# fanxiaochen/Multi-View-Registration

Hardware: AMD Instinct MI355X
Metric: ICP correspondences/sec + ms/iteration, 12-view x 200k pts (higher is better)
Workload: dtype f32

## Files before the change

multi-view-registration_amd/csrc/mvr_ctx.hip:

```cpp
#include <algorithm>
#include <chrono>
#include <cfloat>
#include <cmath>
#include <cstdio>
#include <cstring>

#include "mvr_internal.h"

namespace mvr {

int set_error(Ctx *c, int status, const char *what, hipError_t e)
{
  if (c) {
    c->last_error = what ? what : "";
    if (e != hipSuccess) { c->last_error += ": "; c->last_error += hipGetErrorString(e); }
  }
  return status;
}

void host_mark(const char *what)
{
  static const bool on = std::getenv("MVR_TRACE_HOST") != nullptr;
  if (!on) return;
  using namespace std::chrono;
// ... 922 lines not shown
    if (b > s.n) b = s.n;
    if (n > s.n - b) n = s.n - b;
    if (t.n == 0) n = 0;
    qb[k] = b; qn[k] = n;
    off_s[k + 1] = off_s[k] + s.n; off_t[k + 1] = off_t[k] + t.n;
    off_p[k + 1] = off_p[k] + (size_t)reduce_blocks_for(c, n) * 29;
  }
  const nnkey_t *keys_before = w->bkeys;
  if (int rc = ensure(w, w->bkeys, w->bkeys_cap, off_s[n_pairs])) return rc;
  if (int rc = ensure(w, w->brkeys, w->brkeys_cap, off_t[n_pairs])) return rc;
  const uint32_t *bound_before = w->bbound;
  if (int rc = ensure(w, w->bbound, w->bbound_cap, off_t[n_pairs])) return rc;
  if (w->bbound != bound_before) w->bbound_clean = false;
  if (int rc = ensure(w, w->bpartials, w->bpartials_cap, off_p[n_pairs])) return rc;
  if (int rc = ensure(w, w->blist, w->blist_cap, off_t[n_pairs])) return rc;
  if (int rc = ensure(w, w->bslot, w->bslot_cap, off_t[n_pairs])) return rc;
  std::vector<size_t> off_c((size_t)n_pairs + 1, 0);
  for (int k = 0; k < n_pairs; ++k) off_c[k + 1] = off_c[k] + (c->slots[dst[k]].n + 255) / 256;
  if (int rc = ensure(w, w->bchunks, w->bchunks_cap, off_c[n_pairs] + (size_t)n_pairs)) return rc;
  uint32_t *counts = w->bchunks + off_c[n_pairs];
  const double max2 = max_dist * max_dist;
  const float cap2 = cap_from_max2(max2);
  if ((phases & 2) && c->last_batch.size() >= (size_t)(pair_base + n_pairs))
    for (int k = 0; k < n_pairs; ++k) {
      BatchPairRec &r = c->last_batch[(size_t)(pair_base + k)];
      r.w = w; r.off_s = off_s[k]; r.off_t = off_t[k]; r.qb = qb[k]; r.qn = qn[k]; r.src = src[k]; r.dst = dst[k]; r.max2 = max2; r.reciprocal = reciprocal;
      r.src_set = c->slots[src[k]].set_id; r.dst_set = c->slots[dst[k]].set_id;
    }
  std::vector<unsigned long long> sig;
  sig.push_back((unsigned long long)n_pairs); sig.push_back((unsigned long long)(fma != 0));
  for (int k = 0; k < n_pairs; ++k) {
    const Cloud &s = c->slots[src[k]], &t = c->slots[dst[k]];
    const unsigned long long v[6] = {s.set_id, t.set_id, (unsigned long long)s.n, (unsigned long long)t.n, (unsigned long long)qb[k], (unsigned long long)qn[k]};
    sig.insert(sig.end(), v, v + 6);
  }
  const bool seed = c->seed_forward && (phases & 1) && keys_before == w->bkeys && w->fused_sig == sig;
  if (phases & 1) w->fused_sig = sig;
  std::vector<CullPair> fwd((size_t)n_pairs), rev((size_t)n_pairs);
  for (int k = 0; k < n_pairs; ++k) {
    const Cloud &s = c->slots[src[k]], &t = c->slots[dst[k]];
    fwd[k] = make_cull_pair(s, qb[k], qn[k], nullptr, t, w->bkeys + off_s[k]);
    fwd[k].key_by_pos = 1;
    fwd[k].seed_from_keys = seed ? 1u : 0u;
    rev[k] = make_cull_pair(t, 0, std::min(qn[k], t.n), nullptr, s, w->brkeys + off_t[k]);
    rev[k].qlist = w->blist + off_t[k]; rev[k].qcount = counts + k;
    rev[k].qbound = w->bbound + off_t[k];
  }
  bool grid_ok = c->ring_search != 0 && cap2 < FLT_MAX;
  for (int k = 0; k < n_pairs && grid_ok; ++k) {
    const Cloud &s = c->slots[src[k]], &t = c->slots[dst[k]];
    if (qn[k] == 0) continue;
    grid_ok = s.grid && t.grid && s.gcoords_valid && t.gcoords_valid && s.grid->n == s.n && t.grid->n == t.n &&
              s.order && t.order && s.grid->built_for == s.order.get() && t.grid->built_for == t.order.get();
  }
  std::vector<GridPair> gfwd, grev;
  if (grid_ok) {
    if (int rc = ensure(w, w->bheavy, w->bheavy_cap, off_s[n_pairs] + off_t[n_pairs])) return rc;
    if (int rc = ensure(w, w->bwide, w->bwide_cap, off_s[n_pairs] + off_t[n_pairs])) return rc;
    if (!w->bwide_count) {
      MVR_MAY_BLOCK(w, "the wide-query counters are not allocated yet");
      MVR_HIP_TRY(w, hipMalloc(&w->bwide_count, 3 * kWideCounters * sizeof(uint32_t)));
      MVR_HIP_TRY(w, hipMemsetAsync(w->bwide_count, 0, 3 * kWideCounters * sizeof(uint32_t), w->stream));
    }
    if (int rc = ensure(w, w->bcull_sets, w->bcull_sets_cap, off_s[n_pairs] / 64 + (size_t)n_pairs)) return rc;
    if (n_pairs > kWideCounters) grid_ok = false;
  }
  if (grid_ok) {
    gfwd.resize((size_t)n_pairs); grev.resize((size_t)n_pairs);
    for (int k = 0; k < n_pairs; ++k) {
      const Cloud &s = c->slots[src[k]], &t = c->slots[dst[k]];
      if (qn[k] == 0) { gfwd[k] = GridPair(); grev[k] = GridPair(); continue; }
      gfwd[k] = make_grid_pair(s, qb[k], qn[k], t, w->bkeys + off_s[k]);
      gfwd[k].key_by_pos = 1; gfwd[k].seed_from_keys = seed ? 1u : 0u; gfwd[k].mark = fwd[k].mark;
      gfwd[k].heavy = w->bheavy + off_s[k];
      grev[k] = make_grid_pair(t, 0, std::min(qn[k], t.n), s, w->brkeys + off_t[k]);
      grev[k].qlist = rev[k].qlist; grev[k].qcount = rev[k].qcount; grev[k].qbound = rev[k].qbound;
      grev[k].heavy = w->bheavy + off_s[n_pairs] + off_t[k];
      if (c->cull_list) { gfwd[k].cull_sets = w->bcull_sets + off_s[k] / 64 + (size_t)k; gfwd[k].cull_count = w->bwide_count + 2 * kWideCounters + k; }
      if (c->grid_wide) {
        grev[k].heavy = nullptr;
        gfwd[k].wide_list = w->bwide + off_s[k]; gfwd[k].wide_count = w->bwide_count + k;
        grev[k].wide_list = w->bwide + off_s[n_pairs] + off_t[k]; grev[k].wide_count = w->bwide_count + kWideCounters + k;
      }
    }
  }
  const bool grid_fwd = grid_ok && (seed || c->unseeded_grid);
  bool sets_on_grid = grid_ok && c->cull_list && c->grid_sets;
  if (sets_on_grid && c->grid_sets == 1)
    for (int k = 0; k < n_pairs && sets_on_grid; ++k) {
      if (!qn[k]) continue;
      const double span = (2.0 * max_dist + 4.0) / (double)c->slots[dst[k]].grid->h;
// ... 53 lines not shown
  for (int base = 0; base < n_pairs; base += kBatchPairs) {
    const int m = std::min(kBatchPairs, n_pairs - base);
    GlueBatch gb;
    gb.max2 = max2; gb.reciprocal = recip ? 1 : 0;
    for (int k = 0; k < 3; ++k) gb.origin[k] = origin[k];
    for (int j = 0; j < m; ++j) {
      const int k = base + j;
      const Cloud &s = c->slots[src[k]], &t = c->slots[dst[k]];
      GluePair &g = gb.p[j];
      g.src = s.pts; g.tgt = t.pts; g.qs = s.sorted; g.ts = t.sorted; g.by_pos = 1;
      if (s.sorted_stale) { g.qraw = s.lean_raw; g.qrec = s.pose_dev; }
      if (t.sorted_stale) { g.traw = t.lean_raw; g.trec = t.pose_dev; }
      g.keys = w->bkeys + off_s[k]; g.rkeys = w->brkeys + off_t[k];
      g.qperm = (s.order && qn[k]) ? s.order->perm : nullptr; g.tinv = (t.order && qn[k]) ? t.order->inv : nullptr;
      g.bound = w->bbound + off_t[k];
      g.list = w->blist + off_t[k]; g.slot = w->bslot + off_t[k]; g.chunks = w->bchunks + off_c[k]; g.qcount = counts + k;
      g.nt = qn[k] ? t.n : 0;
      g.partials = w->bpartials + off_p[k]; g.out = table + (size_t)k * 32;
      g.q_begin = qb[k]; g.q_count = qn[k]; g.blocks = reduce_blocks_for(c, qn[k]);
      if (grid_ok) { g.zero_a = w->bwide_count + k; g.zero_b = w->bwide_count + kWideCounters + k; g.zero_c = w->bwide_count + 2 * kWideCounters + k; }
    }
    if (recip) {
      if (!w->marked_in_search) { if (int rc = launch_flag_matched_batch(w, gb, m)) return rc; }
      if (int rc = launch_compact_flags_batch(w, gb, m)) return rc;
      if (grid_ok) {
        if (int rc = launch_nn_grid_batch(w, grev.data() + base, m, cap2, fma != 0)) return rc;
        if (c->grid_debug && c->grid_wide) {
          MVR_MAY_BLOCK(c, "grid_debug reads counters back");
          std::vector<uint32_t> cnt((size_t)2 * kWideCounters), qc((size_t)n_pairs);
          MVR_HIP_TRY(w, hipStreamSynchronize(w->stream));
          MVR_HIP_TRY(w, hipMemcpy(cnt.data(), w->bwide_count, cnt.size() * sizeof(uint32_t), hipMemcpyDeviceToHost));
// ... 151 lines not shown
  if (s.set_id != r.src_set || t.set_id != r.dst_set || !s.order || !t.order)
    return set_error(c, MVR_E_ARG, "the clouds of that pair have changed since the batch");
  MVR_HIP_TRY(c, hipSetDevice(c->device));
  if (r.qn == 0) return MVR_OK;
  Ctx *w = r.w;
  const size_t ns = s.n, nt = t.n;
  std::vector<nnkey_t> keys(r.qn), rkeys(nt);
  std::vector<uint32_t> slot(nt), sperm(ns), tperm(nt);
  MVR_HIP_TRY(c, hipStreamSynchronize(c->stream));
  if (w != c) MVR_HIP_TRY(c, hipStreamSynchronize(w->stream));
  MVR_HIP_TRY(c, hipMemcpy(keys.data(), w->bkeys + r.off_s + r.qb, r.qn * sizeof(nnkey_t), hipMemcpyDeviceToHost));
  MVR_HIP_TRY(c, hipMemcpy(sperm.data(), s.order->perm, ns * 4, hipMemcpyDeviceToHost));
  MVR_HIP_TRY(c, hipMemcpy(tperm.data(), t.order->perm, nt * 4, hipMemcpyDeviceToHost));
  if (r.reciprocal) {
    MVR_HIP_TRY(c, hipMemcpy(rkeys.data(), w->brkeys + r.off_t, nt * sizeof(nnkey_t), hipMemcpyDeviceToHost));
    MVR_HIP_TRY(c, hipMemcpy(slot.data(), w->bslot + r.off_t, nt * 4, hipMemcpyDeviceToHost));
  }
  struct Rec { int32_t q, mt; uint32_t d; };
  std::vector<Rec> acc;
  for (size_t p = 0; p < r.qn; ++p) {
    const nnkey_t key = keys[p];
    const uint32_t tpos = (uint32_t)key, db = (uint32_t)(key >> 32);
    float d; std::memcpy(&d, &db, 4);
    if (tpos == kNone || tpos >= nt || (double)d > r.max2) continue;
    const uint32_t qi = sperm[r.qb + p];
    if (r.reciprocal) {
      const uint32_t li = slot[tpos];
      if (li >= nt) continue;
      const nnkey_t rk = rkeys[li];
      const uint32_t rb = (uint32_t)(rk >> 32);
      float dr; std::memcpy(&dr, &rb, 4);
      if ((uint32_t)rk != qi || (double)dr > r.max2) continue;
    }
    acc.push_back(Rec{(int32_t)qi, (int32_t)tperm[tpos], db});
  }
  std::sort(acc.begin(), acc.end(), [](const Rec &a, const Rec &b) { return a.q < b.q; });
  for (size_t i = 0; i < acc.size() && i < cap; ++i) {
    if (query) query[i] = acc[i].q;
    if (match) match[i] = acc[i].mt;
    if (dist2) std::memcpy(&dist2[i], &acc[i].d, 4);
  }
  *m = acc.size();
// ... 869 lines not shown

API int mvr_ctx_tune(mvr_ctx *ctx, const char *key, int value)
{
  if (!ctx || !key) return MVR_E_ARG;
  Ctx *c = CTX(ctx);
  c->lean_route = false;
  if (!std::strcmp(key, "nn_q")) c->nn_q = value;
  else if (!std::strcmp(key, "nn_sub")) c->nn_sub = value;
  else if (!std::strcmp(key, "nn_blocks_per_cu")) c->nn_blocks_per_cu = value;
  else if (!std::strcmp(key, "nn_mode")) c->nn_mode = value;
  else if (!std::strcmp(key, "cull_q")) c->cull_q = value;
  else if (!std::strcmp(key, "cull_w")) c->cull_w = value;
  else if (!std::strcmp(key, "cull_slices")) c->cull_slices = value;
  else if (!std::strcmp(key, "seed_forward")) c->seed_forward = value != 0;
  else if (!std::strcmp(key, "lean_pose")) { if (value < 0 || value > 1) return MVR_E_ARG; c->lean_pose = value; }
  else if (!std::strcmp(key, "lazy_super")) { if (value < 0 || value > 1) return MVR_E_ARG; c->lazy_super = value; }
  else if (!std::strcmp(key, "fused_mark")) { if (value < 0 || value > 2) return MVR_E_ARG; c->fused_mark = value; }
  else if (!std::strcmp(key, "ring_search")) c->ring_search = value;
  else if (!std::strcmp(key, "seq_search")) { if (value < 0 || value > 1) return MVR_E_ARG; c->seq_search = value; }
  else if (!std::strcmp(key, "unseeded_grid")) { if (value < 0 || value > 1) return MVR_E_ARG; c->unseeded_grid = value; }
  else if (!std::strcmp(key, "seq_cell_points")) { if (value < 1) return MVR_E_ARG; c->seq_cell_points = value; }
  else if (!std::strcmp(key, "seq_seed")) {
    c->seq_seed = value != 0;
    if (!c->seq_seed) {
      MVR_HIP_TRY(c, hipStreamSynchronize(c->stream));
      for (auto &kv : c->seq_seeds) if (kv.second.d) (void)hipFree(kv.second.d);
      c->seq_seeds.clear();
    }
  }
  else if (!std::strcmp(key, "grid_light_rows")) { if (value < 1) return MVR_E_ARG; c->grid_light_rows = value; }
// ... 57 lines not shown
{
  if (!ctx || !n || cap < 0 || (cap && !ms)) return MVR_E_ARG;
  Ctx *c = CTX(ctx);
  *n = (int)c->pass_ms.size();
  for (int k = 0; k < cap && k < *n; ++k) ms[k] = c->pass_ms[(size_t)k];
  return MVR_OK;
}

API int mvr_ctx_stat(mvr_ctx *ctx, const char *key, double *value)
{
  if (!ctx || !key || !value) return MVR_E_ARG;
  Ctx *c = CTX(ctx);
  if (!std::strcmp(key, "piped_passes")) *value = (double)c->piped_passes;
  else if (!std::strcmp(key, "fused_passes")) *value = (double)c->fused_passes;
  else if (!std::strcmp(key, "lean_passes")) *value = (double)c->lean_passes;
  else if (!std::strcmp(key, "blocking_events")) *value = (double)c->blocking_events;
  else if (!std::strcmp(key, "pipeline")) *value = (double)c->pipeline;
  else if (!std::strcmp(key, "prerej_match_ms")) *value = c->prerej_ms[0];
  else if (!std::strcmp(key, "prerej_hypotheses_ms")) *value = c->prerej_ms[1];
  else if (!std::strcmp(key, "prerej_score_ms")) *value = c->prerej_ms[2];
  else if (!std::strncmp(key, "stage_", 6) && c->stage_stat) {
    unsigned long long h[64] = {0};
    std::vector<unsigned long long> raw(64 * 64);
    MVR_HIP_TRY(c, hipStreamSynchronize(c->stream));
    MVR_HIP_TRY(c, hipMemcpy(raw.data(), c->stage_stat, raw.size() * sizeof(unsigned long long), hipMemcpyDeviceToHost));
    for (int sh = 0; sh < 64; ++sh) for (int k = 0; k < 64; ++k) h[k] += raw[(size_t)sh * 64 + k];
    if (!std::strncmp(key, "stage_raw_", 10)) { const int k = std::atoi(key + 10); if (k < 0 || k > 63) return MVR_E_ARG; *value = (double)h[k]; }
    else if (!std::strcmp(key, "stage_staged")) *value = (double)(h[1] + h[9]);
    else if (!std::strcmp(key, "stage_rows")) *value = (double)(h[2] + h[10]);
    else if (!std::strcmp(key, "stage_width")) *value = (double)(h[3] + h[11]);
// ... 92 lines not shown
```

multi-view-registration_amd/csrc/mvr_cull.hip:

```cpp
#include "mvr_internal.h"

namespace mvr {
namespace {

constexpr int kSub = 32;
constexpr int kGrpPitch = 65;

template <bool FMA>
__device__ __forceinline__ float dist2(const float4 t, float qx, float qy, float qz)
{
  const float dx = t.x - qx, dy = t.y - qy, dz = t.z - qz;
  if (FMA) return __builtin_fmaf(dz, dz, __builtin_fmaf(dy, dy, dx * dx));
  float r = dx * dx;
  r = r + dy * dy;
  r = r + dz * dz;
  return r;
}

__device__ __forceinline__ float box_dist2(const float qlo[3], const float qhi[3], const float4 lo, const float4 hi)
{
  const float dx = fmaxf(0.f, fmaxf(lo.x - qhi[0], qlo[0] - hi.x));
  const float dy = fmaxf(0.f, fmaxf(lo.y - qhi[1], qlo[1] - hi.y));
  const float dz = fmaxf(0.f, fmaxf(lo.z - qhi[2], qlo[2] - hi.z));
  return dx * dx + dy * dy + dz * dz;
// ... 39 lines not shown
}

#ifdef MVR_STAMP
#define MVR_CLK() __builtin_readcyclecounter()
#else
#define MVR_CLK() 0ull
#endif

template <bool FMA, int Q, int W>
__device__ __forceinline__ void
nn_cull_body(const float4 *__restrict__ qs, uint32_t q_begin, uint32_t q_count, const uint8_t *__restrict__ qflags,
               const uint32_t *__restrict__ qlist, const uint32_t *__restrict__ qcount, const float4 *__restrict__ ts, uint32_t nt,
               const float4 *__restrict__ tlo, const float4 *__restrict__ thi, const float4 *__restrict__ cbox,
               const float4 *__restrict__ sbox, uint32_t n_tiles, float cap2, nnkey_t *__restrict__ keys, uint32_t key_by_pos,
               const uint32_t *__restrict__ qbound, uint32_t seed_from_keys, uint32_t *__restrict__ mark, uint32_t set,
               unsigned long long *__restrict__ evals)
{
  constexpr int NQ = 4 * Q;
  constexpr int NB = 64 * Q;
  static_assert(W == 1 || W == 2 || W == 4, "waves per query set");
  static_assert(4 * NB * sizeof(nnkey_t) <= 4 * kGrpPitch * sizeof(float4), "partials must fit the tile buffers");
  __shared__ float4 lds[W][4 * kGrpPitch];
  __shared__ unsigned sbest[NB];
  const int lane = threadIdx.x & 63, wv = __builtin_amdgcn_readfirstlane((int)(threadIdx.x >> 6));
  const int g = lane >> 4, l16 = lane & 15;
  const unsigned long long st_entry = MVR_CLK();
#ifdef MVR_TRACE
  const unsigned long long tr_rt0 = __builtin_amdgcn_s_memrealtime();
  unsigned long long trm[8] = {0, 0, 0, 0, 0, 0, 0, 0};
  unsigned trq = 0, tr_open = 0, tr_exp = 0;
  unsigned long long tr_t_open = 0, tr_t_exp = 0, tr_t_next = 0;
// ... 468 lines not shown
#pragma unroll 1
          for (int p = 0; p < 4 * W; ++p) {
            nnkey_t k;
            if constexpr (W == 1) k = (nnkey_t)__shfl(((nnkey_t)__float_as_uint(best[j]) << 32) | bsub[j], p * 16 + l16, 64);
            else k = part[p * NB + i];
            if ((uint32_t)(k >> 32) == dbits && (uint32_t)k != sub && (uint32_t)k != kNone)
              ow = min(ow, span_argmin<FMA, kSub / 4>(ts, nt, (uint32_t)k * kSub + g * (kSub / 4), d, fqx[j], fqy[j], fqz[j]));
          }
        }
      }
      ow = min(ow, (winner_t)__shfl_xor(ow, 16, 64));
      ow = min(ow, (winner_t)__shfl_xor(ow, 32, 64));
      if (g == 0 && pos < nq && (!qflags || qflags[q_begin + pos] != 0)) {
        uint32_t ord = (qlist || (qflags && !key_by_pos)) ? pos : q_begin + pos;
        if (!(qflags || qlist) && !key_by_pos) ord = (W == 1) ? __float_as_uint(qs[q_begin + pos].w) : fqw[j];
        const uint32_t low = key_by_pos ? (uint32_t)ow : (uint32_t)(ow >> 32);
        keys[ord] = (found && ow != kNoWinner) ? (((nnkey_t)dbits << 32) | low) : kKeyInit;
        if (mark && found && ow != kNoWinner) __hip_atomic_store(&mark[low], dbits, __ATOMIC_RELAXED, __HIP_MEMORY_SCOPE_AGENT);
      }
    }
    __builtin_amdgcn_sched_barrier(0);
  }
  MVR_MARK(7);
  if (evals && lane == 0) {
    const unsigned long long e = (unsigned long long)cells_done * 64ull * nvalid;
    unsigned long long *a = evals + (size_t)(set & (kEvalShards - 1)) * kEvalStride;
    unsigned long long *b = a + kEvalRegion;
    atomicAdd(a, e);
    atomicAdd(b, e);
    atomicMax(b + 1, (unsigned long long)cells_done);
// ... 40 lines not shown
#endif
#ifdef MVR_CULL_WAVES_MAX
#define MVR_CULL_WAVES_ATTR MVR_CULL_WAVES, MVR_CULL_WAVES_MAX
#else
#define MVR_CULL_WAVES_ATTR MVR_CULL_WAVES
#endif
template <bool FMA, int Q, int W>
__global__ void __launch_bounds__(64 * W) __attribute__((amdgpu_waves_per_eu(Q == 1 ? (W == 4 ? MVR_CULL_WAVES + 1 : MVR_CULL_WAVES) : 3)))
nn_cull_kernel(CullBatch batch, XcdMap map, unsigned long long *__restrict__ evals)
{
  uint32_t pair = 0, set = 0;
  if (!xcd_map_block(map, blockIdx.x, &pair, &set)) return;
  pair = (uint32_t)__builtin_amdgcn_readfirstlane((int)pair); set = (uint32_t)__builtin_amdgcn_readfirstlane((int)set);
  const CullPair &a = batch.p[pair];
  nn_cull_body<FMA, Q, W>(a.qs, a.q_begin, a.q_count, a.qflags, a.qlist, a.qcount, a.ts, a.nt, a.tlo, a.thi, a.cbox, a.sbox, a.n_tiles, batch.cap2,
                          a.keys, a.key_by_pos, a.qbound, a.seed_from_keys, a.key_by_pos ? a.mark : nullptr, set, evals);
}

template <bool FMA, int W>
__global__ void __launch_bounds__(64 * W)
nn_cull_list_kernel(CullBatch batch, unsigned long long *__restrict__ evals)
{
  const CullPair &a = batch.p[blockIdx.y];
  if (!a.setcount) return;
  const uint32_t n = *a.setcount;
  for (uint32_t i = blockIdx.x; i < n; i += gridDim.x) {
    const uint32_t set = (uint32_t)__builtin_amdgcn_readfirstlane((int)a.setlist[i]);
    nn_cull_body<FMA, 1, W>(a.qs, a.q_begin, a.q_count, a.qflags, a.qlist, a.qcount, a.ts, a.nt, a.tlo, a.thi, a.cbox, a.sbox, a.n_tiles, batch.cap2,
                            a.keys, a.key_by_pos, a.qbound, a.seed_from_keys, a.key_by_pos ? a.mark : nullptr, set, evals);
    __syncthreads();
  }
}

}

int launch_nn_cull_list_batch(Ctx *c, const CullPair *pairs, int n_pairs, float cap2, bool fma)
{
  if (int rc = flush_super_boxes(c)) return rc;
  for (int base = 0; base < n_pairs; base += kBatchPairs) {
    CullBatch batch;
    const int m = std::min(kBatchPairs, n_pairs - base);
    bool any = false;
    for (int k = 0; k < kBatchPairs; ++k) {
      batch.p[k] = k < m ? pairs[base + k] : CullPair{};
// ... 127 lines not shown
```

multi-view-registration_amd/csrc/mvr_grid.hip:

```cpp
#include <hipcub/hipcub.hpp>

#include <algorithm>
#include <cmath>
#include <cstring>
#include <iterator>
#include <type_traits>
#include <vector>

#include "mvr_internal.h"
#include "mvr_grid_size.h"

namespace mvr {

CellGrid::~CellGrid()
{
  if (block) (void)hipFree(block);
  if (ready) (void)hipEventDestroy(ready);
}

namespace {

struct GridGeom { float lo[3]; float inv_h; int dim[3]; };

__device__ __forceinline__ int cell_of(float x, float lo, float inv_h, int dim)
// ... 510 lines not shown
        }
      }
    }
    if (stage_stat && lane == 0 && why) atomicAdd(stage_stat + (size_t)((blockIdx.x * 4u + (uint32_t)wv) & 63u) * 64u + why + (a.qlist ? 8u : 0u), 1ull);
    if (staged) walks = false;
  }
#ifdef MVR_STAGE_CLOCK
  if (!staged) { while (ckn < 4) { ck[ckn] = (long long)__builtin_readcyclecounter(); ++ckn; } }
#endif
  if (walks) walk_box(x0, x1, y0, y1, z0, z1);
  MVR_CK();
  if (answers) {
    const float bd = __uint_as_float((uint32_t)(best >> 32));
    const uint32_t bi = (uint32_t)best;
    const bool found = bi != kNone && bd <= cap2;
    const uint32_t ord = a.qlist ? pos : (a.key_by_pos ? qpos : __float_as_uint(q.w));
    uint32_t low = bi;
    if (found && (a.key_by_pos || a.mark)) {
      const uint32_t hp = a.tinv[bi];
      if (a.key_by_pos) low = hp;
      if (a.mark) __hip_atomic_store(&a.mark[hp], __float_as_uint(bd), __ATOMIC_RELAXED, __HIP_MEMORY_SCOPE_AGENT);
    }
    a.keys[ord] = found ? (((nnkey_t)__float_as_uint(bd) << 32) | low) : kKeyInit;
  }
  if (a.cull_sets) {
    if (__ballot(went_cull) != 0ull && (threadIdx.x & 63) == 0) a.cull_sets[atomicAdd(a.cull_count, 1u)] = (set * kGridThreads + threadIdx.x) >> 6;
  }
  {
    const unsigned long long m = __ballot(went_wide);
    if (m) {
      const int lane = threadIdx.x & 63;
// ... 81 lines not shown
        const nnkey_t key = ((nnkey_t)__float_as_uint(gdist2<FMA>(t, q.x, q.y, q.z)) << 32) | __float_as_uint(t.w);
        if (key < best) { best = key; bk = k; }
      }
      n_eval += total;
      __builtin_amdgcn_fence(__ATOMIC_RELEASE, "wavefront"); __builtin_amdgcn_wave_barrier(); __builtin_amdgcn_fence(__ATOMIC_ACQUIRE, "wavefront");
    }
    nnkey_t m = best;
#pragma unroll
    for (int o = 32; o > 0; o >>= 1) { const nnkey_t v = (nnkey_t)__shfl_xor((unsigned long long)m, o, 64); m = v < m ? v : m; }
    const unsigned long long who = __ballot(best == m && (uint32_t)best != kNone);
    const bool found = (uint32_t)m != kNone && __uint_as_float((uint32_t)(m >> 32)) <= cap2;
    if (found && who) {
      const int src = __ffsll((long long)who) - 1;
      const uint32_t wk = (uint32_t)__shfl((int)bk, src, 64);
      if (lane == 0) {
        const uint32_t ord = a.qlist ? pos : (a.key_by_pos ? qpos : __float_as_uint(q.w));
        uint32_t low = (uint32_t)m;
        if (a.key_by_pos || a.mark) {
          const uint32_t hp = a.g2h[wk];
          if (a.key_by_pos) low = hp;
          if (a.mark) __hip_atomic_store(&a.mark[hp], (uint32_t)(m >> 32), __ATOMIC_RELAXED, __HIP_MEMORY_SCOPE_AGENT);
        }
        a.keys[ord] = (m & 0xFFFFFFFF00000000ull) | low;
      }
    } else if (lane == 0) {
      const uint32_t ord = a.qlist ? pos : (a.key_by_pos ? qpos : __float_as_uint(q.w));
      a.keys[ord] = kKeyInit;
    }
  }
  if (evals && lane == 0 && n_eval) {
    unsigned long long *s = evals + (size_t)((bx * kWideWaves + wv) & (kEvalShards - 1)) * kEvalStride;
    atomicAdd(s, n_eval);
    atomicAdd(s + kEvalRegion, n_eval);
  }
}

}

namespace {
size_t align256(size_t v) { return (v + 255) & ~(size_t)255; }
__global__ void bbox_many_partial_kernel(const float4 *const *__restrict__ pts, const unsigned long long *__restrict__ n, float *__restrict__ part)
// ... 815 lines not shown
```

multi-view-registration_amd/csrc/mvr_index.hip:

```cpp
#include <hipcub/hipcub.hpp>

#include <algorithm>
#include <cstring>
#include <vector>

#include "mvr_internal.h"

namespace mvr {

uint32_t *OrderPool::take(size_t bytes, size_t *got)
{
  int best = -1;
  for (int k = 0; k < (int)free.size(); ++k)
    if (free[k].bytes >= bytes && free[k].bytes <= 4 * bytes + (1u << 20) && (best < 0 || free[k].bytes < free[best].bytes)) best = k;
  if (best < 0) return nullptr;
  uint32_t *p = free[best].p;
  *got = free[best].bytes;
  free.erase(free.begin() + best);
  return p;
}

void OrderPool::give(uint32_t *p, size_t bytes)
{
  if (!p) return;
// ... 337 lines not shown
  if (lane == 0) wsum[wave] = wave_all;
  __syncthreads();
  unsigned before = 0, all = 0;
#pragma unroll
  for (int w = 0; w < kChunk / 64; ++w) { if (w < wave) before += wsum[w]; all += wsum[w]; }
  *total = all;
  return before + mine;
}

__device__ __forceinline__ void chunk_write(const GluePair &a, const unsigned m, const size_t base, const unsigned first)
{
#pragma unroll
  for (int j = 0; j < kChunkPer; ++j)
    if ((m >> j) & 1u) {
      const unsigned at = first + (unsigned)__popc(m & ((1u << j) - 1u));
      a.list[at] = (uint32_t)(base + j); a.slot[base + j] = at;
    }
}

__global__ void __launch_bounds__(kChunk) count_flags_batch_kernel(GlueBatch b)
{
  const GluePair &a = b.p[blockIdx.y];
  if ((size_t)blockIdx.x * kChunkPos >= a.nt) return;
  unsigned total;
  (void)chunk_rank(flagged4(a, (size_t)blockIdx.x * kChunkPos + (size_t)threadIdx.x * kChunkPer), &total);
  if (threadIdx.x == 0) a.chunks[blockIdx.x] = total;
}

constexpr int kScanThreads = 1024;
__global__ void __launch_bounds__(kScanThreads) scan_chunks_batch_kernel(GlueBatch b)
{
// ... 629 lines not shown
```

multi-view-registration_amd/csrc/mvr_internal.h:

```cpp
#pragma once

#include <hip/hip_runtime.h>

#include <algorithm>
#include <cstddef>
#include <cstdint>
#include <map>
#include <memory>
#include <string>
#include <unordered_map>
#include <vector>

#include "mvr_hip.h"

namespace mvr {
hipError_t pool_malloc(void **p, size_t bytes);
hipError_t pool_free(void *p);
hipError_t pool_host_malloc(void **p, size_t bytes, unsigned flags);
hipError_t pool_host_free(void *p);
template <class T> inline hipError_t pool_malloc_t(T **p, size_t bytes) { return pool_malloc(reinterpret_cast<void **>(p), bytes); }
template <class T> inline hipError_t pool_host_malloc_t(T **p, size_t bytes, unsigned flags = 0) { return pool_host_malloc(reinterpret_cast<void **>(p), bytes, flags); }
template <class T> inline hipError_t pool_free_t(T *p) { return pool_free(const_cast<void *>(static_cast<const void *>(p))); }
template <class T> inline hipError_t pool_host_free_t(T *p) { return pool_host_free(const_cast<void *>(static_cast<const void *>(p))); }
}
// ... 97 lines not shown

using nnkey_t = unsigned long long;
constexpr nnkey_t kKeyInit = ~0ull;

constexpr int kNNThreads = 256;
constexpr int kNNTile = 1024;

constexpr int kCullTile = 256;
constexpr int kEvalShards = 64, kEvalStride = 16;
constexpr size_t kEvalRegion = (size_t)kEvalShards * kEvalStride;
constexpr size_t kTraceBlocks = 4096, kTraceRec = 16;

struct ProfRec { int family; hipEvent_t a, b; double work; const uint64_t *h_count; int n_shards; double per_count; };

struct Ctx;
struct BatchPairRec { Ctx *w = nullptr; size_t off_s = 0, off_t = 0, qb = 0, qn = 0; int src = -1, dst = -1; double max2 = 0.0; int reciprocal = 0; unsigned long long src_set = 0, dst_set = 0; };

struct Ctx {
  int device = 0;
  hipStream_t stream = nullptr;
  bool own_stream = false;
  int n_cu = 0;
  struct Cloud *refresh_rider = nullptr;
  int reduce_rows = 0;
  int clock_mhz = 0;
  std::string name;
  std::string last_error;
  Cloud slots[MVR_MAX_SLOTS + 2];
  uint64_t next_set_id = 1;
  std::map<uint64_t, std::weak_ptr<Order> > orders;
  std::map<uint64_t, std::weak_ptr<CellGrid> > grids;
// ... 98 lines not shown
  uint32_t *done_counter = nullptr; uint32_t signal_seq = 0; bool signal_armed = false, signal_sent = false;
  int lazy_super = 1;
  int setup_first = 1;
  int pose_prep_launch = 0;
  const double *pose_in_cur = nullptr; PoseRec *pose_tab_cur = nullptr; int pose_tab_n = 0; bool pose_tab_pending = false;
  uint32_t *gate = nullptr; bool gate_is_signal = false;
  uint32_t *h_done = nullptr, *d_done = nullptr;
  bool pipe_ops_warm = false;
  uint32_t pipe_seq = 0;
  unsigned long long pipe_steady_sig = 0, pipe_steady_events = ~0ull;
  std::vector<double> pass_ms;
  unsigned long long piped_passes = 0;
  int lean_pose = 1;
  bool lean_route = false;
  unsigned long long lean_passes = 0;
  void *comm = nullptr; bool comm_owned = false; int comm_rank = 0, comm_world = 1;
  void **comm_lender = nullptr;
  bool stream_stuck = false;
  bool comm_broken = false;
  int project_world = 0, project_rank = 0;
  double *proj_rows = nullptr; size_t proj_rows_cap = 0, proj_rows_n = 0;
  int wait_timeout_ms = 60000;
  long long dist_pass = 0, inject_fail_at = -1, inject_stall_at = -1;
  uint32_t *h_stall = nullptr, *d_stall = nullptr;
  long long *seq_keys = nullptr; size_t seq_keys_cap = 0;
  double *seq_row = nullptr;
  double *dist_table = nullptr; size_t dist_table_cap = 0;
  bool prof = false;
  unsigned prof_mask = ~0u;
  bool prof_totals = false;
// ... 150 lines not shown
int flush_super_boxes(Ctx *c);
void new_point_set(Ctx *c, Cloud &cl);
void inherit_point_set(Cloud &dst, const Cloud &src);
bool extend_point_set(Ctx *c, Cloud &dst, size_t old_n, const Cloud &src);
constexpr int kBatchPairs = 16;
struct CullPair {
  const float4 *qs = nullptr, *ts = nullptr, *tlo = nullptr, *thi = nullptr, *cbox = nullptr, *sbox = nullptr;
  const uint8_t *qflags = nullptr;
  const uint32_t *qlist = nullptr, *qcount = nullptr;
  nnkey_t *keys = nullptr;
  uint32_t q_begin = 0, q_count = 0, nt = 0, n_tiles = 0;
  const uint32_t *qbound = nullptr;
  uint32_t *mark = nullptr;
  uint32_t key_by_pos = 0;
  uint32_t seed_from_keys = 0;
  const uint32_t *setlist = nullptr, *setcount = nullptr;
};
struct CullBatch { CullPair p[kBatchPairs]; float cap2; };
CullPair make_cull_pair(const Cloud &q, size_t q_begin, size_t q_count, const uint8_t *qflags, const Cloud &t, nnkey_t *keys);
struct XcdMap { uint32_t sets[kBatchPairs]; uint32_t n_pairs, slices; };
__host__ __device__ inline uint32_t slice_len(uint32_t sets, uint32_t slices, uint32_t slice)
{
  return sets > slice ? (sets - slice + slices - 1u) / slices : 0u;
}
__host__ __device__ inline bool xcd_map_block(const XcdMap &m, uint32_t block, uint32_t *pair, uint32_t *set)
{
  uint32_t r = block >> 3;
  for (uint32_t u = block & 7u; u < m.n_pairs * m.slices; u += 8u) {
    const uint32_t p = u / m.slices, sl = u % m.slices, len = slice_len(m.sets[p], m.slices, sl);
    if (r < len) { *pair = p; *set = sl + r * m.slices; return true; }
// ... 22 lines not shown
  const float4 *qs = nullptr;
  const float4 *qraw = nullptr;
  const uint32_t *qlist = nullptr, *qcount = nullptr;
  uint32_t q_begin = 0, q_count = 0;
  const float4 *gts = nullptr;
  const float4 *ts = nullptr;
  const uint32_t *start = nullptr, *g2h = nullptr, *h2g = nullptr, *tinv = nullptr;
  const uint32_t *dir = nullptr, *recs = nullptr;
  int dt_shift = 0, dtdim[3] = {1, 1, 1};
  const uint8_t *dt = nullptr;
  float lo[3] = {0, 0, 0}, inv_h = 1.f, h = 1.f;
  int dim[3] = {1, 1, 1};
  uint8_t *heavy = nullptr;
  double minv[12] = {1, 0, 0, 0, 0, 1, 0, 0, 0, 0, 1, 0};
  uint32_t nt = 0;
  nnkey_t *keys = nullptr;
  const uint32_t *qbound = nullptr;
  uint32_t *mark = nullptr;
  uint32_t key_by_pos = 0, seed_from_keys = 0;
  const PoseRec *pose_dev = nullptr;
  const PoseRec *qpose_dev = nullptr;
  float stretch = 1.f;
  int dt_max = 12;
  uint32_t *wide_list = nullptr, *wide_count = nullptr;
  uint32_t *cull_sets = nullptr, *cull_count = nullptr;
};
constexpr int kGridBatchPairs = 12;
constexpr int kWideCounters = 64;
constexpr int kGridDtMax = 12;
constexpr int kGridLightRows = 24;
// ... 128 lines not shown
```

multi-view-registration_amd/csrc/mvr_reduce.hip:

```cpp
#include "mvr_internal.h"

namespace mvr {

namespace {

struct Vec3d { double x, y, z; };

constexpr int kRT = 256;
constexpr int kMaxBlocks = 1024;

__device__ __forceinline__ double dpp_row_shr(double v, int ctrl)
{
  const unsigned long long b = (unsigned long long)__double_as_longlong(v);
  int lo = (int)(unsigned)b, hi = (int)(unsigned)(b >> 32);
  switch (ctrl) {
    case 1: lo = __builtin_amdgcn_update_dpp(0, lo, 0x111, 0xF, 0xF, true); hi = __builtin_amdgcn_update_dpp(0, hi, 0x111, 0xF, 0xF, true); break;
    case 2: lo = __builtin_amdgcn_update_dpp(0, lo, 0x112, 0xF, 0xF, true); hi = __builtin_amdgcn_update_dpp(0, hi, 0x112, 0xF, 0xF, true); break;
    case 4: lo = __builtin_amdgcn_update_dpp(0, lo, 0x114, 0xF, 0xF, true); hi = __builtin_amdgcn_update_dpp(0, hi, 0x114, 0xF, 0xF, true); break;
    default: lo = __builtin_amdgcn_update_dpp(0, lo, 0x118, 0xF, 0xF, true); hi = __builtin_amdgcn_update_dpp(0, hi, 0x118, 0xF, 0xF, true); break;
  }
  return __longlong_as_double((long long)(((unsigned long long)(unsigned)hi << 32) | (unsigned long long)(unsigned)lo));
}
__device__ __forceinline__ double lane_value(double v, int lane)
{
// ... 313 lines not shown
    const double px = (double)p4.x - o.x, py = (double)p4.y - o.y, pz = (double)p4.z - o.z;
    const double qx = (double)q4.x - o.x, qy = (double)q4.y - o.y, qz = (double)q4.z - o.z;
    acc[0] += 1.0;
    acc[1] += px; acc[2] += py; acc[3] += pz;
    acc[4] += qx; acc[5] += qy; acc[6] += qz;
    acc[7] += px * px; acc[8] += px * py; acc[9] += px * pz; acc[10] += py * py; acc[11] += py * pz; acc[12] += pz * pz;
    acc[13] += qx * qx; acc[14] += qx * qy; acc[15] += qx * qz; acc[16] += qy * qy; acc[17] += qy * qz; acc[18] += qz * qz;
    acc[19] += px * qx; acc[20] += px * qy; acc[21] += px * qz;
    acc[22] += py * qx; acc[23] += py * qy; acc[24] += py * qz;
    acc[25] += pz * qx; acc[26] += pz * qy; acc[27] += pz * qz;
    if (keys) acc[28] += (double)__uint_as_float((uint32_t)(keys[i] >> 32));
  }
  block_partials<29>(acc, partials);
}

template <bool BYPOS>
__device__ __forceinline__ void accept_moments2_body(const float4 *__restrict__ src, const float4 *__restrict__ tgt,
                                                     const nnkey_t *__restrict__ keys, const nnkey_t *__restrict__ rkeys,
                                                     const uint32_t *__restrict__ slot, const uint32_t *__restrict__ qperm,
                                                     const uint32_t *__restrict__ tinv, size_t q_begin, size_t q_count, double max2,
                                                     int reciprocal, Vec3d o, unsigned block, unsigned n_blocks,
                                                     double *__restrict__ partials, const float4 *__restrict__ qraw = nullptr,
                                                     const PoseRec *qrec = nullptr, const float4 *__restrict__ traw = nullptr,
                                                     const PoseRec *trec = nullptr)
{
  Mat44d Tq, Tt;
  if (BYPOS && qraw) Tq = load_pose_uniform(qrec);
  if (BYPOS && traw) Tt = load_pose_uniform(trec);
  double acc[29];
#pragma unroll
  for (int k = 0; k < 29; ++k) acc[k] = 0.0;
// ... 23 lines not shown
    }
#pragma unroll
    for (int u = 0; u < kUn; ++u) {
      j[u] = (uint32_t)key[u];
      d2[u] = __uint_as_float((uint32_t)(key[u] >> 32));
      ok[u] = ok[u] && (j[u] != kNone) && !((double)d2[u] > max2);
      if (BYPOS) i[u] = (size_t)__float_as_uint(p4[u].w);
    }
    if (BYPOS) {
#pragma unroll
      for (int u = 0; u < kUn; ++u) tpos[u] = ok[u] ? j[u] : 0u;
    } else {
#pragma unroll
      for (int u = 0; u < kUn; ++u) tpos[u] = j[u];
    }
    if (reciprocal) {
      uint32_t tj[kUn];
      nnkey_t rk[kUn];
      if (BYPOS) {
#pragma unroll
        for (int u = 0; u < kUn; ++u) tj[u] = tpos[u];
      } else {
#pragma unroll
        for (int u = 0; u < kUn; ++u) { tj[u] = j[u]; if (ok[u] && tinv) tj[u] = tinv[j[u]]; }
      }
      if (slot) {
#pragma unroll
        for (int u = 0; u < kUn; ++u) if (ok[u]) tj[u] = slot[tj[u]];
      }
#pragma unroll
      for (int u = 0; u < kUn; ++u) { rk[u] = 0; if (ok[u]) rk[u] = rkeys[tj[u]]; }
#pragma unroll
      for (int u = 0; u < kUn; ++u) {
        const float dr = __uint_as_float((uint32_t)(rk[u] >> 32));
        ok[u] = ok[u] && ((uint32_t)rk[u] == (uint32_t)i[u]) && !((double)dr > max2);
      }
    }
#pragma unroll
    for (int u = 0; u < kUn; ++u) {
      q4[u] = make_float4(0.f, 0.f, 0.f, 0.f);
      if (ok[u]) { if (!BYPOS) p4[u] = src[i[u]]; q4[u] = (BYPOS && traw) ? traw[tpos[u]] : tgt[tpos[u]]; }
    }
    if (BYPOS && (qraw || traw)) {
#pragma unroll
      for (int u = 0; u < kUn; ++u) {
        if (!ok[u]) continue;
        if (qraw) p4[u] = pose_point_f64(Tq, p4[u]);
        if (traw) q4[u] = pose_point_f64(Tt, q4[u]);
      }
    }
#pragma unroll
    for (int u = 0; u < kUn; ++u) {
      if (!ok[u]) continue;
      const double px = (double)p4[u].x - o.x, py = (double)p4[u].y - o.y, pz = (double)p4[u].z - o.z;
      const double qx = (double)q4[u].x - o.x, qy = (double)q4[u].y - o.y, qz = (double)q4[u].z - o.z;
      acc[0] += 1.0;
// ... 16 lines not shown
                       const uint32_t *__restrict__ tinv, size_t q_begin, size_t q_count, double max2, int reciprocal, Vec3d o,
                       double *__restrict__ partials)
{
  accept_moments2_body<false>(src, tgt, keys, rkeys, slot, qperm, tinv, q_begin, q_count, max2, reciprocal, o, blockIdx.x, gridDim.x, partials);
}

__global__ void __launch_bounds__(kRT) accept_moments2_batch_kernel(GlueBatch b)
{
  const GluePair &a = b.p[blockIdx.y];
  if ((int)blockIdx.x >= a.blocks) return;
  if (blockIdx.x == 0 && threadIdx.x == 0) { if (a.zero_a) *a.zero_a = 0u; if (a.zero_b) *a.zero_b = 0u; if (a.zero_c) *a.zero_c = 0u; }
  if (a.bound && b.reciprocal)
    for (unsigned long long i = (unsigned long long)blockIdx.x * blockDim.x + threadIdx.x; i < a.nt; i += (unsigned long long)a.blocks * blockDim.x)
      a.bound[i] = 0xFFFFFFFFu;
  const Vec3d o{b.origin[0], b.origin[1], b.origin[2]};
  if (a.by_pos)
    accept_moments2_body<true>(a.qs, a.ts, a.keys, a.rkeys, a.slot, nullptr, a.tinv, (size_t)a.q_begin, (size_t)a.q_count, b.max2, b.reciprocal, o,
                               blockIdx.x, (unsigned)a.blocks, a.partials, a.qraw, a.qrec, a.traw, a.trec);
  else
    accept_moments2_body<false>(a.src, a.tgt, a.keys, a.rkeys, a.slot, a.qperm, a.tinv, (size_t)a.q_begin, (size_t)a.q_count, b.max2, b.reciprocal, o,
                                blockIdx.x, (unsigned)a.blocks, a.partials);
}

__global__ void __launch_bounds__(kRT) moments2_final_kernel(const double *__restrict__ partials, int rows, Vec3d o,
                                                              double *__restrict__ out)
{
  __shared__ double lds[29];
  double s[29];
  sum_rows<29>(partials, rows, s, lds);
  if (threadIdx.x == 0) {
    out[0] = s[0]; out[1] = o.x; out[2] = o.y; out[3] = o.z;
// ... 367 lines not shown
```

Baseline: 7.716 billion.

## Key reverse NN results by target position to drop slot indirection

The reverse nearest-neighbour kernels (cull and grid) can now write their keys indexed by the target's sorted position instead of by compact list index. This lets the accept/moments kernel read rkeys directly at tpos, skipping the slot-array write in the list builder and the dependent slot gather at accept time. The change is on by default through a new accept_chain option and also updates the debug verification path. In exchange, the brkeys writes become scattered rather than compact, and the path relies on brkeys being sized for the full target cloud.

```diff
diff --git a/multi-view-registration_amd/csrc/mvr_ctx.hip b/multi-view-registration_amd/csrc/mvr_ctx.hip
--- a/multi-view-registration_amd/csrc/mvr_ctx.hip
+++ b/multi-view-registration_amd/csrc/mvr_ctx.hip
@@ -960,7 +960,9 @@
   if (w->bbound != bound_before) w->bbound_clean = false;
   if (int rc = ensure(w, w->bpartials, w->bpartials_cap, off_p[n_pairs])) return rc;
   if (int rc = ensure(w, w->blist, w->blist_cap, off_t[n_pairs])) return rc;
-  if (int rc = ensure(w, w->bslot, w->bslot_cap, off_t[n_pairs])) return rc;
+  const bool chain2 = c->accept_chain != 0;
+  if (!chain2) { if (int rc = ensure(w, w->bslot, w->bslot_cap, off_t[n_pairs])) return rc; }
+  if (chain2 && reciprocal && (phases & 2) && pair_base == 0) ++c->accept_chain_passes;
   std::vector<size_t> off_c((size_t)n_pairs + 1, 0);
   for (int k = 0; k < n_pairs; ++k) off_c[k + 1] = off_c[k] + (c->slots[dst[k]].n + 255) / 256;
   if (int rc = ensure(w, w->bchunks, w->bchunks_cap, off_c[n_pairs] + (size_t)n_pairs)) return rc;
@@ -970,7 +972,7 @@
   if ((phases & 2) && c->last_batch.size() >= (size_t)(pair_base + n_pairs))
     for (int k = 0; k < n_pairs; ++k) {
       BatchPairRec &r = c->last_batch[(size_t)(pair_base + k)];
-      r.w = w; r.off_s = off_s[k]; r.off_t = off_t[k]; r.qb = qb[k]; r.qn = qn[k]; r.src = src[k]; r.dst = dst[k]; r.max2 = max2; r.reciprocal = reciprocal;
+      r.w = w; r.off_s = off_s[k]; r.off_t = off_t[k]; r.qb = qb[k]; r.qn = qn[k]; r.src = src[k]; r.dst = dst[k]; r.max2 = max2; r.reciprocal = reciprocal; r.rkeys_by_tpos = chain2;
       r.src_set = c->slots[src[k]].set_id; r.dst_set = c->slots[dst[k]].set_id;
     }
   std::vector<unsigned long long> sig;
@@ -989,7 +991,7 @@
     fwd[k].key_by_pos = 1;
     fwd[k].seed_from_keys = seed ? 1u : 0u;
     rev[k] = make_cull_pair(t, 0, std::min(qn[k], t.n), nullptr, s, w->brkeys + off_t[k]);
-    rev[k].qlist = w->blist + off_t[k]; rev[k].qcount = counts + k;
+    rev[k].qlist = w->blist + off_t[k]; rev[k].qcount = counts + k; rev[k].key_by_qpos = chain2 ? 1u : 0u;
     rev[k].qbound = w->bbound + off_t[k];
   }
   bool grid_ok = c->ring_search != 0 && cap2 < FLT_MAX;
@@ -1020,7 +1022,7 @@
       gfwd[k].key_by_pos = 1; gfwd[k].seed_from_keys = seed ? 1u : 0u; gfwd[k].mark = fwd[k].mark;
       gfwd[k].heavy = w->bheavy + off_s[k];
       grev[k] = make_grid_pair(t, 0, std::min(qn[k], t.n), s, w->brkeys + off_t[k]);
-      grev[k].qlist = rev[k].qlist; grev[k].qcount = rev[k].qcount; grev[k].qbound = rev[k].qbound;
+      grev[k].qlist = rev[k].qlist; grev[k].qcount = rev[k].qcount; grev[k].qbound = rev[k].qbound; grev[k].key_by_qpos = rev[k].key_by_qpos;
       grev[k].heavy = w->bheavy + off_s[n_pairs] + off_t[k];
       if (c->cull_list) { gfwd[k].cull_sets = w->bcull_sets + off_s[k] / 64 + (size_t)k; gfwd[k].cull_count = w->bwide_count + 2 * kWideCounters + k; }
       if (c->grid_wide) {
@@ -1104,7 +1106,7 @@
       g.keys = w->bkeys + off_s[k]; g.rkeys = w->brkeys + off_t[k];
       g.qperm = (s.order && qn[k]) ? s.order->perm : nullptr; g.tinv = (t.order && qn[k]) ? t.order->inv : nullptr;
       g.bound = w->bbound + off_t[k];
-      g.list = w->blist + off_t[k]; g.slot = w->bslot + off_t[k]; g.chunks = w->bchunks + off_c[k]; g.qcount = counts + k;
+      g.list = w->blist + off_t[k]; g.slot = chain2 ? nullptr : w->bslot + off_t[k]; g.chunks = w->bchunks + off_c[k]; g.qcount = counts + k;
       g.nt = qn[k] ? t.n : 0;
       g.partials = w->bpartials + off_p[k]; g.out = table + (size_t)k * 32;
       g.q_begin = qb[k]; g.q_count = qn[k]; g.blocks = reduce_blocks_for(c, qn[k]);
@@ -1286,7 +1288,7 @@
   MVR_HIP_TRY(c, hipMemcpy(tperm.data(), t.order->perm, nt * 4, hipMemcpyDeviceToHost));
   if (r.reciprocal) {
     MVR_HIP_TRY(c, hipMemcpy(rkeys.data(), w->brkeys + r.off_t, nt * sizeof(nnkey_t), hipMemcpyDeviceToHost));
-    MVR_HIP_TRY(c, hipMemcpy(slot.data(), w->bslot + r.off_t, nt * 4, hipMemcpyDeviceToHost));
+    if (!r.rkeys_by_tpos) MVR_HIP_TRY(c, hipMemcpy(slot.data(), w->bslot + r.off_t, nt * 4, hipMemcpyDeviceToHost));
   }
   struct Rec { int32_t q, mt; uint32_t d; };
   std::vector<Rec> acc;
@@ -1297,7 +1299,7 @@
     if (tpos == kNone || tpos >= nt || (double)d > r.max2) continue;
     const uint32_t qi = sperm[r.qb + p];
     if (r.reciprocal) {
-      const uint32_t li = slot[tpos];
+      const uint32_t li = r.rkeys_by_tpos ? tpos : slot[tpos];
       if (li >= nt) continue;
       const nnkey_t rk = rkeys[li];
       const uint32_t rb = (uint32_t)(rk >> 32);
@@ -2197,6 +2199,7 @@
   else if (!std::strcmp(key, "cull_slices")) c->cull_slices = value;
   else if (!std::strcmp(key, "seed_forward")) c->seed_forward = value != 0;
   else if (!std::strcmp(key, "lean_pose")) { if (value < 0 || value > 1) return MVR_E_ARG; c->lean_pose = value; }
+  else if (!std::strcmp(key, "accept_chain")) { if (value < 0 || value > 1) return MVR_E_ARG; c->accept_chain = value; }
   else if (!std::strcmp(key, "lazy_super")) { if (value < 0 || value > 1) return MVR_E_ARG; c->lazy_super = value; }
   else if (!std::strcmp(key, "fused_mark")) { if (value < 0 || value > 2) return MVR_E_ARG; c->fused_mark = value; }
   else if (!std::strcmp(key, "ring_search")) c->ring_search = value;
@@ -2284,6 +2287,7 @@
   if (!std::strcmp(key, "piped_passes")) *value = (double)c->piped_passes;
   else if (!std::strcmp(key, "fused_passes")) *value = (double)c->fused_passes;
   else if (!std::strcmp(key, "lean_passes")) *value = (double)c->lean_passes;
+  else if (!std::strcmp(key, "accept_chain_passes")) *value = (double)c->accept_chain_passes;
   else if (!std::strcmp(key, "blocking_events")) *value = (double)c->blocking_events;
   else if (!std::strcmp(key, "pipeline")) *value = (double)c->pipeline;
   else if (!std::strcmp(key, "prerej_match_ms")) *value = c->prerej_ms[0];
diff --git a/multi-view-registration_amd/csrc/mvr_cull.hip b/multi-view-registration_amd/csrc/mvr_cull.hip
--- a/multi-view-registration_amd/csrc/mvr_cull.hip
+++ b/multi-view-registration_amd/csrc/mvr_cull.hip
@@ -77,7 +77,7 @@
                const float4 *__restrict__ tlo, const float4 *__restrict__ thi, const float4 *__restrict__ cbox,
                const float4 *__restrict__ sbox, uint32_t n_tiles, float cap2, nnkey_t *__restrict__ keys, uint32_t key_by_pos,
                const uint32_t *__restrict__ qbound, uint32_t seed_from_keys, uint32_t *__restrict__ mark, uint32_t set,
-               unsigned long long *__restrict__ evals)
+               unsigned long long *__restrict__ evals, uint32_t key_by_qpos = 0)
 {
   constexpr int NQ = 4 * Q;
   constexpr int NB = 64 * Q;
@@ -576,6 +576,7 @@
       if (g == 0 && pos < nq && (!qflags || qflags[q_begin + pos] != 0)) {
         uint32_t ord = (qlist || (qflags && !key_by_pos)) ? pos : q_begin + pos;
         if (!(qflags || qlist) && !key_by_pos) ord = (W == 1) ? __float_as_uint(qs[q_begin + pos].w) : fqw[j];
+        if (qlist && key_by_qpos) ord = qlist[pos];
         const uint32_t low = key_by_pos ? (uint32_t)ow : (uint32_t)(ow >> 32);
         keys[ord] = (found && ow != kNoWinner) ? (((nnkey_t)dbits << 32) | low) : kKeyInit;
         if (mark && found && ow != kNoWinner) __hip_atomic_store(&mark[low], dbits, __ATOMIC_RELAXED, __HIP_MEMORY_SCOPE_AGENT);
@@ -646,7 +647,7 @@
   pair = (uint32_t)__builtin_amdgcn_readfirstlane((int)pair); set = (uint32_t)__builtin_amdgcn_readfirstlane((int)set);
   const CullPair &a = batch.p[pair];
   nn_cull_body<FMA, Q, W>(a.qs, a.q_begin, a.q_count, a.qflags, a.qlist, a.qcount, a.ts, a.nt, a.tlo, a.thi, a.cbox, a.sbox, a.n_tiles, batch.cap2,
-                          a.keys, a.key_by_pos, a.qbound, a.seed_from_keys, a.key_by_pos ? a.mark : nullptr, set, evals);
+                          a.keys, a.key_by_pos, a.qbound, a.seed_from_keys, a.key_by_pos ? a.mark : nullptr, set, evals, a.key_by_qpos);
 }
 
 template <bool FMA, int W>
@@ -659,7 +660,7 @@
   for (uint32_t i = blockIdx.x; i < n; i += gridDim.x) {
     const uint32_t set = (uint32_t)__builtin_amdgcn_readfirstlane((int)a.setlist[i]);
     nn_cull_body<FMA, 1, W>(a.qs, a.q_begin, a.q_count, a.qflags, a.qlist, a.qcount, a.ts, a.nt, a.tlo, a.thi, a.cbox, a.sbox, a.n_tiles, batch.cap2,
-                            a.keys, a.key_by_pos, a.qbound, a.seed_from_keys, a.key_by_pos ? a.mark : nullptr, set, evals);
+                            a.keys, a.key_by_pos, a.qbound, a.seed_from_keys, a.key_by_pos ? a.mark : nullptr, set, evals, a.key_by_qpos);
     __syncthreads();
   }
 }
diff --git a/multi-view-registration_amd/csrc/mvr_grid.hip b/multi-view-registration_amd/csrc/mvr_grid.hip
--- a/multi-view-registration_amd/csrc/mvr_grid.hip
+++ b/multi-view-registration_amd/csrc/mvr_grid.hip
@@ -548,7 +548,7 @@
     const float bd = __uint_as_float((uint32_t)(best >> 32));
     const uint32_t bi = (uint32_t)best;
     const bool found = bi != kNone && bd <= cap2;
-    const uint32_t ord = a.qlist ? pos : (a.key_by_pos ? qpos : __float_as_uint(q.w));
+    const uint32_t ord = a.qlist ? (a.key_by_qpos ? qpos : pos) : (a.key_by_pos ? qpos : __float_as_uint(q.w));
     uint32_t low = bi;
     if (found && (a.key_by_pos || a.mark)) {
       const uint32_t hp = a.tinv[bi];
@@ -660,7 +660,7 @@
       const int src = __ffsll((long long)who) - 1;
       const uint32_t wk = (uint32_t)__shfl((int)bk, src, 64);
       if (lane == 0) {
-        const uint32_t ord = a.qlist ? pos : (a.key_by_pos ? qpos : __float_as_uint(q.w));
+        const uint32_t ord = a.qlist ? (a.key_by_qpos ? qpos : pos) : (a.key_by_pos ? qpos : __float_as_uint(q.w));
         uint32_t low = (uint32_t)m;
         if (a.key_by_pos || a.mark) {
           const uint32_t hp = a.g2h[wk];
@@ -670,7 +670,7 @@
         a.keys[ord] = (m & 0xFFFFFFFF00000000ull) | low;
       }
     } else if (lane == 0) {
-      const uint32_t ord = a.qlist ? pos : (a.key_by_pos ? qpos : __float_as_uint(q.w));
+      const uint32_t ord = a.qlist ? (a.key_by_qpos ? qpos : pos) : (a.key_by_pos ? qpos : __float_as_uint(q.w));
       a.keys[ord] = kKeyInit;
     }
   }
diff --git a/multi-view-registration_amd/csrc/mvr_index.hip b/multi-view-registration_amd/csrc/mvr_index.hip
--- a/multi-view-registration_amd/csrc/mvr_index.hip
+++ b/multi-view-registration_amd/csrc/mvr_index.hip
@@ -375,7 +375,8 @@
   for (int j = 0; j < kChunkPer; ++j)
     if ((m >> j) & 1u) {
       const unsigned at = first + (unsigned)__popc(m & ((1u << j) - 1u));
-      a.list[at] = (uint32_t)(base + j); a.slot[base + j] = at;
+      a.list[at] = (uint32_t)(base + j);
+      if (a.slot) a.slot[base + j] = at;
     }
 }
 
diff --git a/multi-view-registration_amd/csrc/mvr_internal.h b/multi-view-registration_amd/csrc/mvr_internal.h
--- a/multi-view-registration_amd/csrc/mvr_internal.h
+++ b/multi-view-registration_amd/csrc/mvr_internal.h
@@ -135,7 +135,7 @@
 struct ProfRec { int family; hipEvent_t a, b; double work; const uint64_t *h_count; int n_shards; double per_count; };
 
 struct Ctx;
-struct BatchPairRec { Ctx *w = nullptr; size_t off_s = 0, off_t = 0, qb = 0, qn = 0; int src = -1, dst = -1; double max2 = 0.0; int reciprocal = 0; unsigned long long src_set = 0, dst_set = 0; };
+struct BatchPairRec { Ctx *w = nullptr; size_t off_s = 0, off_t = 0, qb = 0, qn = 0; int src = -1, dst = -1; double max2 = 0.0; int reciprocal = 0; unsigned long long src_set = 0, dst_set = 0; bool rkeys_by_tpos = false; };
 
 struct Ctx {
   int device = 0;
@@ -264,6 +264,8 @@
   int lean_pose = 1;
   bool lean_route = false;
   unsigned long long lean_passes = 0;
+  int accept_chain = 1;
+  unsigned long long accept_chain_passes = 0;
   void *comm = nullptr; bool comm_owned = false; int comm_rank = 0, comm_world = 1;
   void **comm_lender = nullptr;
   bool stream_stuck = false;
@@ -444,6 +446,7 @@
   uint32_t *mark = nullptr;
   uint32_t key_by_pos = 0;
   uint32_t seed_from_keys = 0;
+  uint32_t key_by_qpos = 0;
   const uint32_t *setlist = nullptr, *setcount = nullptr;
 };
 struct CullBatch { CullPair p[kBatchPairs]; float cap2; };
@@ -496,6 +499,7 @@
   uint8_t *heavy = nullptr;
   double minv[12] = {1, 0, 0, 0, 0, 1, 0, 0, 0, 0, 1, 0};
   uint32_t nt = 0;
+  uint32_t key_by_qpos = 0;
   nnkey_t *keys = nullptr;
   const uint32_t *qbound = nullptr;
   uint32_t *mark = nullptr;
diff --git a/multi-view-registration_amd/csrc/mvr_reduce.hip b/multi-view-registration_amd/csrc/mvr_reduce.hip
--- a/multi-view-registration_amd/csrc/mvr_reduce.hip
+++ b/multi-view-registration_amd/csrc/mvr_reduce.hip
@@ -351,7 +351,7 @@
   block_partials<29>(acc, partials);
 }
 
-template <bool BYPOS>
+template <bool BYPOS, bool CHAIN2 = false>
 __device__ __forceinline__ void accept_moments2_body(const float4 *__restrict__ src, const float4 *__restrict__ tgt,
                                                      const nnkey_t *__restrict__ keys, const nnkey_t *__restrict__ rkeys,
                                                      const uint32_t *__restrict__ slot, const uint32_t *__restrict__ qperm,
@@ -405,6 +405,22 @@
 #pragma unroll
       for (int u = 0; u < kUn; ++u) tpos[u] = j[u];
     }
+    if constexpr (CHAIN2) {
+      static_assert(BYPOS, "the two-stage chain reads sorted space");
+      nnkey_t rk[kUn];
+#pragma unroll
+      for (int u = 0; u < kUn; ++u) {
+        rk[u] = 0; q4[u] = make_float4(0.f, 0.f, 0.f, 0.f);
+        if (ok[u]) { if (reciprocal) rk[u] = rkeys[tpos[u]]; q4[u] = traw ? traw[tpos[u]] : tgt[tpos[u]]; }
+      }
+      if (reciprocal) {
+#pragma unroll
+        for (int u = 0; u < kUn; ++u) {
+          const float dr = __uint_as_float((uint32_t)(rk[u] >> 32));
+          ok[u] = ok[u] && ((uint32_t)rk[u] == (uint32_t)i[u]) && !((double)dr > max2);
+        }
+      }
+    } else {
     if (reciprocal) {
       uint32_t tj[kUn];
       nnkey_t rk[kUn];
@@ -431,6 +447,7 @@
     for (int u = 0; u < kUn; ++u) {
       q4[u] = make_float4(0.f, 0.f, 0.f, 0.f);
       if (ok[u]) { if (!BYPOS) p4[u] = src[i[u]]; q4[u] = (BYPOS && traw) ? traw[tpos[u]] : tgt[tpos[u]]; }
+    }
     }
     if (BYPOS && (qraw || traw)) {
 #pragma unroll
@@ -477,7 +494,10 @@
     for (unsigned long long i = (unsigned long long)blockIdx.x * blockDim.x + threadIdx.x; i < a.nt; i += (unsigned long long)a.blocks * blockDim.x)
       a.bound[i] = 0xFFFFFFFFu;
   const Vec3d o{b.origin[0], b.origin[1], b.origin[2]};
-  if (a.by_pos)
+  if (a.by_pos && !a.slot)
+    accept_moments2_body<true, true>(a.qs, a.ts, a.keys, a.rkeys, nullptr, nullptr, a.tinv, (size_t)a.q_begin, (size_t)a.q_count, b.max2, b.reciprocal, o,
+                                     blockIdx.x, (unsigned)a.blocks, a.partials, a.qraw, a.qrec, a.traw, a.trec);
+  else if (a.by_pos)
     accept_moments2_body<true>(a.qs, a.ts, a.keys, a.rkeys, a.slot, nullptr, a.tinv, (size_t)a.q_begin, (size_t)a.q_count, b.max2, b.reciprocal, o,
                                blockIdx.x, (unsigned)a.blocks, a.partials, a.qraw, a.qrec, a.traw, a.trec);
   else
```

Measured after the change: 7.730 billion, median of 2. No clear change (+0.2%).
